# twice154/ofa-for-super-resolution

Measured on AMD Instinct MI355X. Metric: sr_training_images_per_sec_4x_64to256, higher is better.
Workload: dtype bf16; 1 GPU; OFA-SR S4 supernet 4x progressive shrinking (elastic kernel {3,5,7}, e=6, d=4, pd=2), LR 64x64 -> HR 256x256, fwd+bwd+Adam, train-mode BN; kernel_transform_mode=1, compat_reference_indexing=True, parallelism=dp1, per_gpu_batch=16, global_batch=16, grad_allreduce_bytes=0, launch=eager

## Files before the change

### ofa-for-super-resolution_amd/csrc/pwconv.hip

```cpp
#include <stdlib.h>
#include "ofasr_common.h"

namespace ofasr {

typedef __attribute__((ext_vector_type(16))) float f32x16;
typedef __attribute__((ext_vector_type(8))) __bf16 bf16x8;
typedef __attribute__((ext_vector_type(8))) _Float16 f16x8;
typedef __attribute__((ext_vector_type(4))) short s16x4;
typedef __attribute__((ext_vector_type(8))) short s16x8;
typedef __attribute__((address_space(3))) s16x4 lds_s16x4;

constexpr int PW_THREADS = 256;
constexpr int PW_TILE = 128;
constexpr int XROW16 = 320;
constexpr int XROW32 = 512;
constexpr int WROW16 = 128;
constexpr int WROW32 = 256;

template <typename T> struct Mma16;
template <> struct Mma16<bf16_t> {
    static __device__ __forceinline__ f32x16 run(s16x8 a, s16x8 b, f32x16 c) {
        return __builtin_amdgcn_mfma_f32_32x32x16_bf16(__builtin_bit_cast(bf16x8, a), __builtin_bit_cast(bf16x8, b),
                                                       c, 0, 0, 0);
    }
// ... 1177 lines not shown

template <typename T> struct Rows64 {
    static constexpr int NIT = Elem<T>::is16 ? 2 : 4;
    static constexpr int CPR = Elem<T>::is16 ? 8 : 16;
    static constexpr int EPC = Elem<T>::is16 ? 8 : 4;
    uint4 v[NIT];
    uint32_t ok;
};
template <typename T>
__device__ __forceinline__ void rows64_request(Rows64<T>& g, const T* __restrict__ base, int rows_total, int r0, int HW, int p0) {
    const int tid = threadIdx.x;
    g.ok = 0;
#pragma unroll
    for (int it = 0; it < Rows64<T>::NIT; ++it) {
        const int q = tid + it * PW_THREADS;
        const int r = q / Rows64<T>::CPR, ch = q % Rows64<T>::CPR;
        const int px = p0 + Rows64<T>::EPC * ch;
        const bool ok = r0 + r < rows_total && px < HW;
        g.v[it] = *reinterpret_cast<const uint4*>(base + (ok ? (long long)(r0 + r) * HW + px : 0));
        g.ok |= (ok ? 1u : 0u) << it;
    }
}
template <typename T>
__device__ __forceinline__ void rows64_deposit(char* Lt, const Rows64<T>& g) {
    const int tid = threadIdx.x;
#pragma unroll
    for (int it = 0; it < Rows64<T>::NIT; ++it) {
        const int q = tid + it * PW_THREADS;
        const int r = q / Rows64<T>::CPR, ch = q % Rows64<T>::CPR;
        const uint32_t m = (g.ok >> it) & 1u ? 0xffffffffu : 0u;
        *reinterpret_cast<uint4*>(Lt + wtile_chunk_off<T>(r, ch)) = make_uint4(g.v[it].x & m, g.v[it].y & m, g.v[it].z & m, g.v[it].w & m);
    }
}

template <typename T, bool ALIGNED>
__global__ void __launch_bounds__(PW_THREADS) pw_wgrad_kernel(const T* __restrict__ R, const T* __restrict__ S,
                                                              float* __restrict__ part, int MR, int NS, int HW,
                                                              int stages_per_img, int total_stages,
                                                              int stages_per_split) {
    constexpr int SUB = WgStage<T>::SUB;
    constexpr int TB = 64 * Elem<T>::wrow;
    __shared__ __attribute__((aligned(16))) char Rt[SUB * TB];
    __shared__ __attribute__((aligned(16))) char St[SUB * TB];
    const int r0 = blockIdx.x * 64, s0 = blockIdx.y * 64, z = blockIdx.z;
    const int lane = lane_id();
    const int wave = __builtin_amdgcn_readfirstlane((int)(threadIdx.x >> 6));
    const int c = lane & 31, h = lane >> 5;
    const int rb = wave & 1, sb = wave >> 1;
    f32x16 acc = zero16();
    const int q_lo = z * stages_per_split;
    const int q_hi = min(total_stages, q_lo + stages_per_split);
    auto multiply = [&]() {
#pragma unroll
        for (int sub = 0; sub < SUB; ++sub) {
            const char* Rs = Rt + sub * TB;
            const char* Ss = St + sub * TB;
            if constexpr (Elem<T>::is16) {
#pragma unroll
                for (int s = 0; s < 4; ++s) {
                    const s16x8 af = *reinterpret_cast<const s16x8*>(Rs + wtile_chunk_off<T>(32 * rb + c, 2 * s + h));
                    const s16x8 bf = *reinterpret_cast<const s16x8*>(Ss + wtile_chunk_off<T>(32 * sb + c, 2 * s + h));
                    acc = Mma16<T>::run(af, bf, acc);
                }
            } else {
#pragma unroll
                for (int s4 = 0; s4 < 8; ++s4) {
                    const float4 a4 = *reinterpret_cast<const float4*>(Rs + wtile_chunk_off<T>(32 * rb + c, 8 * h + s4));
                    const float4 b4 = *reinterpret_cast<const float4*>(Ss + wtile_chunk_off<T>(32 * sb + c, 8 * h + s4));
                    acc = __builtin_amdgcn_mfma_f32_32x32x2f32(a4.x, b4.x, acc, 0, 0, 0);
                    acc = __builtin_amdgcn_mfma_f32_32x32x2f32(a4.y, b4.y, acc, 0, 0, 0);
                    acc = __builtin_amdgcn_mfma_f32_32x32x2f32(a4.z, b4.z, acc, 0, 0, 0);
                    acc = __builtin_amdgcn_mfma_f32_32x32x2f32(a4.w, b4.w, acc, 0, 0, 0);
                }
            }
        }
    };
    if constexpr (ALIGNED) {
        Rows64<T> rg[SUB], sg[SUB];
        auto request = [&](int q) {
            const int n = q / stages_per_img;
            const int p0 = (q - n * stages_per_img) * (64 * SUB);
#pragma unroll
            for (int sub = 0; sub < SUB; ++sub) {
                rows64_request<T>(rg[sub], R + (long long)n * MR * HW, MR, r0, HW, p0 + 64 * sub);
                rows64_request<T>(sg[sub], S + (long long)n * NS * HW, NS, s0, HW, p0 + 64 * sub);
            }
        };
        if (q_lo < q_hi) request(q_lo);
        for (int q = q_lo; q < q_hi; ++q) {
            if (q > q_lo) __syncthreads();
#pragma unroll
            for (int sub = 0; sub < SUB; ++sub) {
                rows64_deposit<T>(Rt + sub * TB, rg[sub]);
                rows64_deposit<T>(St + sub * TB, sg[sub]);
            }
            __syncthreads();
            if (q + 1 < q_hi) request(q + 1);
            multiply();
        }
    } else {
        for (int q = q_lo; q < q_hi; ++q) {
            const int n = q / stages_per_img;
            const int p0 = (q - n * stages_per_img) * (64 * SUB);
            if (q > q_lo) __syncthreads();
#pragma unroll
            for (int sub = 0; sub < SUB; ++sub) {
                stage_rows64<T, ALIGNED>(Rt + sub * TB, R + (long long)n * MR * HW, MR, r0, HW, p0 + 64 * sub);
                stage_rows64<T, ALIGNED>(St + sub * TB, S + (long long)n * NS * HW, NS, s0, HW, p0 + 64 * sub);
            }
            __syncthreads();
            multiply();
        }
    }
    float* pz = part + (long long)z * MR * NS;
    const int sc = s0 + 32 * sb + c;
#pragma unroll
    for (int reg = 0; reg < 16; ++reg) {
        const int rr = r0 + 32 * rb + acc_row(reg, h);
        if (rr < MR && sc < NS) pz[(long long)rr * NS + sc] = acc[reg];
    }
}

constexpr int WR_ZL = 16;
__global__ void __launch_bounds__(64 * WR_ZL) pw_wgrad_reduce_kernel(const float* __restrict__ part,
                                                                     float* __restrict__ dw, int MR, int NS, int nsplit,
                                                                     long long sr, long long ss) {
    __shared__ float red[WR_ZL][64];
    const long long tot = (long long)MR * NS;
    const long long idx = (long long)blockIdx.x * 64 + (threadIdx.x & 63);
    const int zl = threadIdx.x >> 6;
    float a = 0.f;
    if (idx < tot) {
        int z = zl;
        for (; z + 3 * WR_ZL < nsplit; z += 4 * WR_ZL) {
            const float v0 = part[(long long)z * tot + idx], v1 = part[(long long)(z + WR_ZL) * tot + idx];
            const float v2 = part[(long long)(z + 2 * WR_ZL) * tot + idx], v3 = part[(long long)(z + 3 * WR_ZL) * tot + idx];
            a += (v0 + v1) + (v2 + v3);
        }
        for (; z < nsplit; z += WR_ZL) a += part[(long long)z * tot + idx];
    }
    red[zl][threadIdx.x & 63] = a;
    __syncthreads();
    if (zl == 0 && idx < tot) {
        float t = 0.f;
#pragma unroll
        for (int i = 0; i < WR_ZL; ++i) t += red[i][threadIdx.x];
        const long long r = idx / NS, sx = idx - r * NS;
        dw[r * sr + sx * ss] = t;
    }
}

constexpr int WD_RB = 3;
constexpr int WD_ROWS = 4 * WD_RB * 32, WD_COLS = 64;

struct WdPlan {
    int quads_per_img, total_quads, nsplit, MR, NS;
};

template <typename T, int XF = 0>
__global__ void __launch_bounds__(512) pw_wgrad_direct_kernel(const T* __restrict__ R, const T* __restrict__ S,
                                                              float* __restrict__ part, int MR, int NS, int HW,
                                                              WdPlan wp, InputXf xf = InputXf{}, BwdXf bx = BwdXf{}) {
    const int lane = lane_id();
    const int wave = __builtin_amdgcn_readfirstlane((int)(threadIdx.x >> 6));
    const int wr = wave & 3, wc = wave >> 2;
    const int c = lane & 31, h = lane >> 5;
    const int split = blockIdx.x;
    const int row0 = blockIdx.y * WD_ROWS + wr * (WD_RB * 32);
    const int col = blockIdx.z * WD_COLS + wc * 32 + c;
    if (row0 >= MR) return;
    f32x16 acc[WD_RB];
#pragma unroll
    for (int rb = 0; rb < WD_RB; ++rb) acc[rb] = zero16();
    const int q0 = (int)((long long)split * wp.total_quads / wp.nsplit);
    const int q1 = (int)((long long)(split + 1) * wp.total_quads / wp.nsplit);
    const bool cs = col < NS;
    const int colc = cs ? col : NS - 1;
    bool rs[WD_RB];
    int rowc[WD_RB];
#pragma unroll
    for (int rb = 0; rb < WD_RB; ++rb) {
        rs[rb] = row0 + 32 * rb + c < MR;
        rowc[rb] = rs[rb] ? row0 + 32 * rb + c : MR - 1;
    }
    float xsc[WD_RB], xmu[WD_RB], xb[WD_RB];
    float csc = 1.f, cmu = 0.f, cbb = 0.f;
    if constexpr (XF == 1) {
#pragma unroll
        for (int rb = 0; rb < WD_RB; ++rb) {
            xsc[rb] = xf.scale[rowc[rb]];
            xmu[rb] = xf.mean[rowc[rb]];
            xb[rb] = fmaf(xmu[rb], xsc[rb], xf.shift[rowc[rb]]);
        }
    }
    if constexpr (XF == 2) {
        csc = xf.scale[colc];
        cmu = xf.mean[colc];
        cbb = fmaf(cmu, csc, xf.shift[colc]);
    }
    float bka[WD_RB], bkbi[WD_RB];
    if constexpr (XF == 3) {
#pragma unroll
        for (int rb = 0; rb < WD_RB; ++rb) {
            xsc[rb] = bx.scale[rowc[rb]];
            xmu[rb] = bx.mean[rowc[rb]];
            xb[rb] = fmaf(xmu[rb], xsc[rb], bx.shift[rowc[rb]]);
            bka[rb] = bx.ka[rowc[rb]];
            bkbi[rb] = bx.kbi[rowc[rb]];
        }
    }
    long long rowoff[WD_RB];
#pragma unroll
    for (int rb = 0; rb < WD_RB; ++rb) rowoff[rb] = (long long)rowc[rb] * HW;
    const long long coloff = (long long)colc * HW;
    for (int q = q0; q < q1; ++q) {
        const int n = q / wp.quads_per_img;
        const int px = (q - n * wp.quads_per_img) * 64 + 32 * h;
        uint4 a[WD_RB][4], b[4];
        bool okp[4];
        int pxc[4];
#pragma unroll
        for (int j = 0; j < 4; ++j) {
            okp[j] = px + 8 * j < HW;
            pxc[j] = okp[j] ? px + 8 * j : 0;
        }
        const T* sp = S + (long long)n * NS * HW + coloff;
#pragma unroll
        for (int j = 0; j < 4; ++j) b[j] = *reinterpret_cast<const uint4*>(sp + pxc[j]);
        const T* rn = R + (long long)n * MR * HW;
#pragma unroll
        for (int rb = 0; rb < WD_RB; ++rb) {
#pragma unroll
            for (int j = 0; j < 4; ++j) {
                a[rb][j] = *reinterpret_cast<const uint4*>(rn + rowoff[rb] + pxc[j]);
            }
        }
        uint4 ya[XF == 3 ? WD_RB : 1][4];
        if constexpr (XF == 3) {
            const T* yn = reinterpret_cast<const T*>(bx.y) + (long long)n * MR * HW;
#pragma unroll
            for (int rb = 0; rb < WD_RB; ++rb) {
#pragma unroll
                for (int j = 0; j < 4; ++j)
                    ya[rb][j] = *reinterpret_cast<const uint4*>(yn + rowoff[rb] + pxc[j]);
            }
        }
#pragma unroll
        for (int j = 0; j < 4; ++j) {
            if constexpr (XF == 2) b[j] = xf_apply8_core<T>(b[j], csc, cmu, cbb);
            if (!(cs && okp[j])) b[j] = make_uint4(0, 0, 0, 0);
        }
#pragma unroll
        for (int rb = 0; rb < WD_RB; ++rb)
#pragma unroll
            for (int j = 0; j < 4; ++j) {
                if constexpr (XF == 1) a[rb][j] = xf_apply8_core<T>(a[rb][j], xsc[rb], xmu[rb], xb[rb]);
                if constexpr (XF == 3) a[rb][j] = bx_apply8<T>(a[rb][j], ya[rb][j], xmu[rb], xsc[rb], xb[rb], bka[rb], bkbi[rb]);
                if (!(rs[rb] && okp[j])) a[rb][j] = make_uint4(0, 0, 0, 0);
            }
#pragma unroll
        for (int j = 0; j < 4; ++j)
#pragma unroll
            for (int rb = 0; rb < WD_RB; ++rb)
                acc[rb] = Mma16<T>::run(__builtin_bit_cast(s16x8, a[rb][j]), __builtin_bit_cast(s16x8, b[j]), acc[rb]);
    }
    float* dst = part + (long long)split * MR * NS;
    if (cs) {
        float* p = dst + (long long)(row0 + 4 * h) * NS + col;
#pragma unroll
        for (int rb = 0; rb < WD_RB; ++rb)
#pragma unroll
            for (int reg = 0; reg < 16; ++reg) {
                const int r = row0 + 32 * rb + acc_row(reg, h);
                if (r < MR) *p = acc[rb][reg];
                p += (reg & 3) == 3 ? 5 * (long long)NS : (long long)NS;
            }
    }
}

static WdPlan wd_plan(int64_t N, int64_t Cin, int64_t Cout, int64_t HW) {
    WdPlan p;
    p.MR = (int)(Cout >= Cin ? Cout : Cin);
    p.NS = (int)(Cout >= Cin ? Cin : Cout);
    p.quads_per_img = (int)cdiv(HW, 64);
    p.total_quads = (int)(N * p.quads_per_img);
    const int64_t tiles = cdiv(p.MR, WD_ROWS) * cdiv(p.NS, WD_COLS);
    static const int blocks = [] { const char* e = getenv("OFASR_PW_WGRAD_BLOCKS"); const int v = e ? atoi(e) : 0; return v > 0 ? v : 256; }();
    int64_t want = blocks / (tiles > 0 ? tiles : 1);
    if (want > p.total_quads / 4) want = p.total_quads / 4;
    if (want < 1) want = 1;
    p.nsplit = (int)want;
    return p;
}


struct WdPlan32 {
    int units_per_img, total_units, nsplit, MR, NS;
};

__global__ void __launch_bounds__(512) pw_wgrad_direct_f32_kernel(const float* __restrict__ R, const float* __restrict__ S,
                                                                  float* __restrict__ part, int MR, int NS, int HW,
                                                                  WdPlan32 wp) {
    const int lane = lane_id();
    const int wave = __builtin_amdgcn_readfirstlane((int)(threadIdx.x >> 6));
    const int wr = wave & 3, wc = wave >> 2;
    const int c = lane & 31, h = lane >> 5;
    const int split = blockIdx.x;
    const int row0 = blockIdx.y * WD_ROWS + wr * (WD_RB * 32);
    const int col = blockIdx.z * WD_COLS + wc * 32 + c;
    if (row0 >= MR) return;
    f32x16 acc[WD_RB];
#pragma unroll
    for (int rb = 0; rb < WD_RB; ++rb) acc[rb] = zero16();
    const int u0 = (int)((long long)split * wp.total_units / wp.nsplit);
    const int u1 = (int)((long long)(split + 1) * wp.total_units / wp.nsplit);
    const bool cs = col < NS;
    const int colc = cs ? col : NS - 1;
    bool rs[WD_RB];
    long long rowoff[WD_RB];
#pragma unroll
    for (int rb = 0; rb < WD_RB; ++rb) {
        rs[rb] = row0 + 32 * rb + c < MR;
        rowoff[rb] = (long long)(rs[rb] ? row0 + 32 * rb + c : MR - 1) * HW;
    }
    float4 a[2][WD_RB][4], b[2][4];
    auto request = [&](int set, int u) {
        const int uc = u < u1 ? u : u1 - 1;
        const int n = uc / wp.units_per_img;
        const int px = (uc - n * wp.units_per_img) * 32 + 16 * h;
        int pxc[4];
#pragma unroll
        for (int j = 0; j < 4; ++j) pxc[j] = px + 4 * j < HW ? px + 4 * j : 0;
        const float* sp = S + ((long long)n * NS + colc) * HW;
        const float* rp = R + (long long)n * MR * HW;
#pragma unroll
        for (int j = 0; j < 4; ++j) b[set][j] = *reinterpret_cast<const float4*>(sp + pxc[j]);
#pragma unroll
        for (int rb = 0; rb < WD_RB; ++rb)
#pragma unroll
            for (int j = 0; j < 4; ++j) a[set][rb][j] = *reinterpret_cast<const float4*>(rp + rowoff[rb] + pxc[j]);
    };
    auto multiply = [&](int set, int u) {
        const int n = u / wp.units_per_img;
        const int px = (u - n * wp.units_per_img) * 32 + 16 * h;
        const bool live = u < u1;
#pragma unroll
        for (int j = 0; j < 4; ++j) {
            const bool ok = live && cs && px + 4 * j < HW;
            const float4 bv = ok ? b[set][j] : make_float4(0.f, 0.f, 0.f, 0.f);
#pragma unroll
            for (int rb = 0; rb < WD_RB; ++rb) {
                const float4 av = rs[rb] ? a[set][rb][j] : make_float4(0.f, 0.f, 0.f, 0.f);
                acc[rb] = __builtin_amdgcn_mfma_f32_32x32x2f32(av.x, bv.x, acc[rb], 0, 0, 0);
                acc[rb] = __builtin_amdgcn_mfma_f32_32x32x2f32(av.y, bv.y, acc[rb], 0, 0, 0);
                acc[rb] = __builtin_amdgcn_mfma_f32_32x32x2f32(av.z, bv.z, acc[rb], 0, 0, 0);
                acc[rb] = __builtin_amdgcn_mfma_f32_32x32x2f32(av.w, bv.w, acc[rb], 0, 0, 0);
            }
        }
    };
    if (u0 < u1) {
        request(0, u0);
        for (int u = u0; u < u1; u += 2) {
            request(1, u + 1);
            multiply(0, u);
            request(0, u + 2);
            multiply(1, u + 1);
        }
    }
    float* dst = part + (long long)split * MR * NS;
    if (cs) {
        float* p = dst + (long long)(row0 + 4 * h) * NS + col;
#pragma unroll
        for (int rb = 0; rb < WD_RB; ++rb)
#pragma unroll
            for (int reg = 0; reg < 16; ++reg) {
                const int r = row0 + 32 * rb + acc_row(reg, h);
                if (r < MR) *p = acc[rb][reg];
                p += (reg & 3) == 3 ? 5 * (long long)NS : (long long)NS;
            }
    }
}

static WdPlan32 wd_plan32(int64_t N, int64_t Cin, int64_t Cout, int64_t HW) {
    WdPlan32 p;
    p.MR = (int)(Cout >= Cin ? Cout : Cin);
    p.NS = (int)(Cout >= Cin ? Cin : Cout);
    p.units_per_img = (int)cdiv(HW, 32);
    p.total_units = (int)(N * p.units_per_img);
    const int64_t tiles = cdiv(p.MR, WD_ROWS) * cdiv(p.NS, WD_COLS);
    int64_t want = 256 / (tiles > 0 ? tiles : 1);
    if (want > p.total_units / 8) want = p.total_units / 8;
    if (want < 1) want = 1;
    p.nsplit = (int)want;
    return p;
}

struct WgradPlan {
    int stages_per_img, total_stages, nsplit, stages_per_split, MR, NS;
};

static WgradPlan wgrad_plan(int64_t N, int64_t Cin, int64_t Cout, int64_t HW, int sub) {
    WgradPlan p;
    p.MR = (int)(Cout >= Cin ? Cout : Cin);
    p.NS = (int)(Cout >= Cin ? Cin : Cout);
    p.stages_per_img = (int)cdiv(HW, 64 * sub);
    p.total_stages = (int)(N * p.stages_per_img);
    const int64_t tiles = cdiv(p.MR, 64) * cdiv(p.NS, 64);
    int64_t want = 512 / (tiles > 0 ? tiles : 1);
    if (want < 1) want = 1;
    if (want > p.total_stages) want = p.total_stages;
    if (want < 1) want = 1;
    p.stages_per_split = (int)cdiv(p.total_stages, want);
    if (p.stages_per_split < 1) p.stages_per_split = 1;
    p.nsplit = (int)cdiv(p.total_stages, p.stages_per_split);
    if (p.nsplit < 1) p.nsplit = 1;
    return p;
}

static bool aligned_for(const void* a, const void* b, int64_t HW, bool is16) {
    const uintptr_t bits = reinterpret_cast<uintptr_t>(a) | reinterpret_cast<uintptr_t>(b);
    return (bits & 15) == 0 && (HW % (is16 ? 8 : 4)) == 0;
}

template <typename T, bool AL, bool WV, bool XF = false>
static void launch_gemm_v(const void* x, WView wv, void* y, int64_t HW, int tiles_per_img, int total_tiles,
                          hipStream_t st, InputXf xf = InputXf{}, const void* addend = nullptr,
                          StatOut so = StatOut{nullptr, 0}, BnFold fold = BnFold{}) {
    if (wv.K <= 64) {
        if constexpr (Elem<T>::is16 && AL && WV && !XF) {
            static const bool slabs = [] { const char* e = getenv("OFASR_PW_FANOUT_SLABS"); return !(e && e[0] == '0'); }();
            const int nslab = wv.M / FO_ROWS;
            if (slabs && addend == nullptr && wv.K == 64 && wv.M % FO_ROWS == 0 && (nslab == 2 || nslab == 3) &&
                HW % PW_TILE == 0) {
                dim3 g1((unsigned)total_tiles);
#define OFASR_FO_SLABS(NS, ST)                                                                                       \
    OFASR_LAUNCH((pw_fanout_slabs_kernel<T, NS, ST>), g1, dim3(PW_THREADS), 0, st, (const T*)x, wv, (T*)y, (int)HW, \
                       tiles_per_img, so, BwdStatOut{})
                if (nslab == 3) { if (so.partial) OFASR_FO_SLABS(3, 1); else OFASR_FO_SLABS(3, 0); }
                else { if (so.partial) OFASR_FO_SLABS(2, 1); else OFASR_FO_SLABS(2, 0); }
#undef OFASR_FO_SLABS
                return;
            }
        }
        dim3 grid((unsigned)total_tiles, (unsigned)cdiv(wv.M, FO_ROWS));
        OFASR_LAUNCH((pw_fanout_kernel<T, AL, WV, XF>), grid, dim3(PW_THREADS), 0, st, (const T*)x, wv, (T*)y,
                           (int)HW, tiles_per_img, xf, (const T*)addend, so);
    } else {
        dim3 grid((unsigned)total_tiles, (unsigned)cdiv(wv.M, 64));
        if constexpr (Elem<T>::is16 && AL && WV) {
            static const bool fast_ok = [] { const char* e = getenv("OFASR_PW_FANIN_FAST"); return !(e && e[0] == '0'); }();
            const bool span32 = (long long)wv.K * HW < (1LL << 31) &&
                                (long long)wv.M * wv.sm + (long long)wv.K * wv.sk < (1LL << 31);
            if (fast_ok && wv.K % 4 == 0 && wv.M % 4 == 0 && span32)
                OFASR_LAUNCH((pw_fanin_pipe_kernel<T, XF, true>), grid, dim3(PW_THREADS), 0, st, (const T*)x, wv,
                                   (T*)y, (int)HW, tiles_per_img, (int)cdiv(wv.K, 64), xf, (const T*)addend, so, fold);
            else
                OFASR_LAUNCH((pw_fanin_pipe_kernel<T, XF, false>), grid, dim3(PW_THREADS), 0, st, (const T*)x, wv,
                                   (T*)y, (int)HW, tiles_per_img, (int)cdiv(wv.K, 64), xf, (const T*)addend, so, fold);
            return;
        }
        OFASR_LAUNCH((pw_fanin_kernel<T, AL, WV, XF>), grid, dim3(PW_THREADS), 0, st, (const T*)x, wv, (T*)y,
                           (int)HW, tiles_per_img, (int)cdiv(wv.K, 64), xf, (const T*)addend, so);
    }
}

template <typename T, bool XF = false>
static int launch_gemm(const char* name, const void* x, WView wv, void* y, int64_t N, int64_t HW, hipStream_t st,
                       InputXf xf = InputXf{}, const void* addend = nullptr, StatOut so = StatOut{nullptr, 0},
                       BnFold fold = BnFold{}) {
    constexpr bool is16 = Elem<T>::is16;
    const bool al = aligned_for(x, y, HW, is16);
    const long long ld = wv.sk == 1 ? wv.sm : wv.sk;
    const bool wvec = (reinterpret_cast<uintptr_t>(wv.w) & 15) == 0 && (ld % 4) == 0 && wv.K % 4 == 0 && wv.M % 4 == 0;
    const int tiles_per_img = (int)cdiv(HW, PW_TILE);
    const int64_t total64 = N * tiles_per_img;
    OFASR_REQUIRE(total64 <= INT32_MAX, OFASR_ERR_UNSUPPORTED, "%s: too many pixel tiles", name);
    const int total_tiles = (int)total64;
    {
        const double px = (double)N * (double)HW, es = (double)sizeof(T);
        prof_note(es * px * (wv.K + wv.M + (addend ? wv.M : 0)) + 4.0 * wv.K * wv.M, 2.0 * px * wv.K * wv.M);
    }
    if (so.partial)
        OFASR_REQUIRE(so.P == (wv.K <= 64 ? total_tiles : 2 * total_tiles), OFASR_ERR_INVALID_ARG,
                      "%s: statistics unit count %d does not match the launch", name, so.P);
    if constexpr (XF) {
        OFASR_REQUIRE(al && is16, OFASR_ERR_UNSUPPORTED, "%s: fused input transform needs aligned 16-bit tensors", name);
        if (fold.cp)
            OFASR_REQUIRE(wvec && wv.K > 64 && wv.K <= FOLD_KMAX, OFASR_ERR_UNSUPPORTED,
                          "%s: folded statistics need the pipelined fan-in kernel (64 < K <= %d)", name, FOLD_KMAX);
        if (wvec) launch_gemm_v<T, true, true, true>(x, wv, y, HW, tiles_per_img, total_tiles, st, xf, nullptr, so, fold);
        else launch_gemm_v<T, true, false, true>(x, wv, y, HW, tiles_per_img, total_tiles, st, xf, nullptr, so);
        return check_launch(name);
    }
    const bool al2 = al && (addend == nullptr || (reinterpret_cast<uintptr_t>(addend) & 15) == 0);
    if (al2 && wvec) launch_gemm_v<T, true, true>(x, wv, y, HW, tiles_per_img, total_tiles, st, InputXf{}, addend, so);
    else if (al2) launch_gemm_v<T, true, false>(x, wv, y, HW, tiles_per_img, total_tiles, st, InputXf{}, addend, so);
    else if (wvec) launch_gemm_v<T, false, true>(x, wv, y, HW, tiles_per_img, total_tiles, st, InputXf{}, addend, so);
    else launch_gemm_v<T, false, false>(x, wv, y, HW, tiles_per_img, total_tiles, st, InputXf{}, addend, so);
    return check_launch(name);
}

static int gemm_entry(const char* name, const void* x, WView wv, void* y, int64_t N, int64_t HW, int dtype,
                      void* stream, const void* addend = nullptr, StatOut so = StatOut{nullptr, 0}) {
    hipStream_t st = as_stream(stream);
    switch (dtype) {
        case OFASR_F32: return launch_gemm<float>(name, x, wv, y, N, HW, st, InputXf{}, addend, so);
        case OFASR_F16: return launch_gemm<f16_t>(name, x, wv, y, N, HW, st, InputXf{}, addend, so);
        default: return launch_gemm<bf16_t>(name, x, wv, y, N, HW, st, InputXf{}, addend, so);
    }
}

static int check_pw_args(const char* name, const void* a, const void* b, const void* c, int64_t ldw, int64_t N,
                         int64_t Cin, int64_t Cout, int64_t HW, int dtype) {
    OFASR_REQUIRE(a && b && c, OFASR_ERR_INVALID_ARG, "%s: null pointer", name);
    OFASR_REQUIRE(N >= 0 && Cin > 0 && Cout > 0 && HW >= 0, OFASR_ERR_INVALID_ARG,
                  "%s: bad shape N=%lld Cin=%lld Cout=%lld HW=%lld", name, (long long)N, (long long)Cin,
                  (long long)Cout, (long long)HW);
    OFASR_REQUIRE(ldw >= Cin, OFASR_ERR_INVALID_ARG, "%s: ldw=%lld < Cin=%lld", name, (long long)ldw, (long long)Cin);
    OFASR_REQUIRE(dtype == OFASR_F32 || dtype == OFASR_F16 || dtype == OFASR_BF16, OFASR_ERR_INVALID_ARG,
                  "%s: bad dtype %d", name, dtype);
    OFASR_REQUIRE(Cin <= 65536 && Cout <= 65536 && HW <= (1 << 30) && N <= (1 << 24), OFASR_ERR_UNSUPPORTED,
                  "%s: dimension too large", name);
    return OFASR_OK;
}

template <typename T, bool XF = false, bool BXM = false>
static int launch_wgrad(const char* name, const void* dy, const void* x, float* dw, int64_t ldw, int64_t N, int64_t Cin,
                        int64_t Cout, int64_t HW, float* ws, hipStream_t st, InputXf xf = InputXf{}, BwdXf bx = BwdXf{}) {
    const WgradPlan p = wgrad_plan(N, Cin, Cout, HW, WgStage<T>::SUB);
    const bool big_is_dy = Cout >= Cin;
    const T* R = (const T*)(big_is_dy ? dy : x);
    const T* S = (const T*)(big_is_dy ? x : dy);
    const long long sr = big_is_dy ? ldw : 1, ss = big_is_dy ? 1 : ldw;
    const bool al = aligned_for(dy, x, HW, Elem<T>::is16);
    prof_note((double)sizeof(T) * (double)N * (double)HW * (double)(Cin + Cout) + 4.0 * (double)Cin * (double)Cout,
              2.0 * (double)N * (double)HW * (double)Cin * (double)Cout);
    if constexpr (Elem<T>::is16) {
        if (al) {
            const WdPlan wp = wd_plan(N, Cin, Cout, HW);
            dim3 grid((unsigned)wp.nsplit, (unsigned)cdiv(wp.MR, WD_ROWS), (unsigned)cdiv(wp.NS, WD_COLS));
            if constexpr (XF) {
                if (big_is_dy)
                    OFASR_LAUNCH((pw_wgrad_direct_kernel<T, 2>), grid, dim3(512), 0, st, R, S, ws, wp.MR, wp.NS,
                                       (int)HW, wp, xf);
                else
                    OFASR_LAUNCH((pw_wgrad_direct_kernel<T, 1>), grid, dim3(512), 0, st, R, S, ws, wp.MR, wp.NS,
                                       (int)HW, wp, xf);
            } else if constexpr (BXM) {
                if (!big_is_dy) {
                    set_error("%s: the fused BN backward is implemented for the wide gradient operand (Cout >= Cin)", name);
                    return OFASR_ERR_UNSUPPORTED;
                }
                OFASR_LAUNCH((pw_wgrad_direct_kernel<T, 3>), grid, dim3(512), 0, st, R, S, ws, wp.MR, wp.NS, (int)HW, wp,
                             InputXf{}, bx);
            } else {
                OFASR_LAUNCH((pw_wgrad_direct_kernel<T>), grid, dim3(512), 0, st, R, S, ws, wp.MR, wp.NS, (int)HW,
                                   wp);
            }
            int rc = check_launch(name);
            if (rc) return rc;
            const long long tot = (long long)wp.MR * wp.NS;
            OFASR_LAUNCH(pw_wgrad_reduce_kernel, dim3((unsigned)cdiv(tot, 64)), dim3(64 * WR_ZL), 0, st, ws, dw, wp.MR,
                               wp.NS, wp.nsplit, sr, ss);
            return check_launch(name);
        }
    }
    if constexpr (XF || BXM) {
        set_error("%s: fused input transform needs the aligned 16-bit kernel", name);
        return OFASR_ERR_UNSUPPORTED;
    }
    if constexpr (!Elem<T>::is16) {
        static const bool f32_direct = [] { const char* e = getenv("OFASR_PW_WGRAD_F32_DIRECT"); return e && e[0] == '1'; }();
        if (al && f32_direct) {
            const WdPlan32 wp = wd_plan32(N, Cin, Cout, HW);
            dim3 grid((unsigned)wp.nsplit, (unsigned)cdiv(wp.MR, WD_ROWS), (unsigned)cdiv(wp.NS, WD_COLS));
            OFASR_LAUNCH(pw_wgrad_direct_f32_kernel, grid, dim3(512), 0, st, (const float*)R, (const float*)S, ws, wp.MR, wp.NS,
                         (int)HW, wp);
            int rc = check_launch(name);
            if (rc) return rc;
            const long long tot = (long long)wp.MR * wp.NS;
            OFASR_LAUNCH(pw_wgrad_reduce_kernel, dim3((unsigned)cdiv(tot, 64)), dim3(64 * WR_ZL), 0, st, ws, dw, wp.MR, wp.NS,
                         wp.nsplit, sr, ss);
            return check_launch(name);
        }
    }
    dim3 grid((unsigned)cdiv(p.MR, 64), (unsigned)cdiv(p.NS, 64), (unsigned)p.nsplit);
    if (al)
        OFASR_LAUNCH((pw_wgrad_kernel<T, true>), grid, dim3(PW_THREADS), 0, st, R, S, ws, p.MR, p.NS, (int)HW,
                           p.stages_per_img, p.total_stages, p.stages_per_split);
    else
        OFASR_LAUNCH((pw_wgrad_kernel<T, false>), grid, dim3(PW_THREADS), 0, st, R, S, ws, p.MR, p.NS, (int)HW,
                           p.stages_per_img, p.total_stages, p.stages_per_split);
    int rc = check_launch(name);
    if (rc) return rc;
    const long long tot = (long long)p.MR * p.NS;
    OFASR_LAUNCH(pw_wgrad_reduce_kernel, dim3((unsigned)cdiv(tot, 64)), dim3(64 * WR_ZL), 0, st, ws, dw, p.MR, p.NS,
                       p.nsplit, sr, ss);
    return check_launch(name);
}

int pwconv_dgrad_add(const void* dy, const float* w, int64_t ldw, void* dx, const void* addend, int64_t N, int64_t Cin,
                     int64_t Cout, int64_t HW, int dtype, void* stream) {
    const char* name = "pwconv_dgrad_add";
    int rc = check_pw_args(name, dy, w, dx, ldw, N, Cin, Cout, HW, dtype);
    if (rc) return rc;
    OFASR_REQUIRE(addend != nullptr, OFASR_ERR_INVALID_ARG, "%s: null addend", name);
    if (N * HW == 0) return OFASR_OK;
    WView wv{w, 1, ldw, (int)Cin, (int)Cout};
    return gemm_entry(name, dy, wv, dx, N, HW, dtype, stream, addend);
}

bool pwconv_dgrad_bx_supported(const void* da, const void* y, const void* dx, const void* addend, const float* w,
                               int64_t ldw, int64_t Cin, int64_t Cout, int64_t HW, int dtype) {
    if (dtype != OFASR_F16 && dtype != OFASR_BF16) return false;
    const uintptr_t bits = reinterpret_cast<uintptr_t>(da) | reinterpret_cast<uintptr_t>(y) | reinterpret_cast<uintptr_t>(dx) |
                           reinterpret_cast<uintptr_t>(addend) | reinterpret_cast<uintptr_t>(w);
    static const bool fast_ok = [] { const char* e = getenv("OFASR_PW_FANIN_FAST"); return !(e && e[0] == '0'); }();
    return fast_ok && (bits & 15) == 0 && HW % 8 == 0 && ldw % 4 == 0 && Cin % 4 == 0 && Cout % 4 == 0 && Cout > 64 &&
           Cout <= FOLD_KMAX && Cout * HW < (1LL << 31) && (Cin + Cout) * ldw < (1LL << 31);
}

template <typename T>
static int launch_dgrad_bx(const char* name, const void* da, WView wv, void* dx, const void* addend, int64_t N, int64_t HW,
                           BwdXf bx, hipStream_t st) {
    const int tiles_per_img = (int)cdiv(HW, PW_TILE);
    const int64_t total64 = N * tiles_per_img;
    OFASR_REQUIRE(total64 <= INT32_MAX, OFASR_ERR_UNSUPPORTED, "%s: too many pixel tiles", name);
    {
        const double px = (double)N * (double)HW, es = (double)sizeof(T);
        prof_note(es * px * (2.0 * wv.K + wv.M + (addend ? wv.M : 0)) + 4.0 * wv.K * wv.M, 2.0 * px * wv.K * wv.M);
    }
    dim3 grid((unsigned)total64, (unsigned)cdiv(wv.M, 64));
    OFASR_LAUNCH((pw_fanin_pipe_kernel<T, false, true, true>), grid, dim3(PW_THREADS), 0, st, (const T*)da, wv, (T*)dx,
                 (int)HW, tiles_per_img, (int)cdiv(wv.K, 64), InputXf{}, (const T*)addend, StatOut{nullptr, 0}, BnFold{}, bx);
    return check_launch(name);
}

int pwconv_dgrad_add_bx(const void* da, const float* w, int64_t ldw, void* dx, const void* addend, int64_t N, int64_t Cin,
                        int64_t Cout, int64_t HW, int dtype, BwdXf bx, void* stream) {
    const char* name = "pwconv_dgrad_add_bx";
    int rc = check_pw_args(name, da, w, dx, ldw, N, Cin, Cout, HW, dtype);
    if (rc) return rc;
    OFASR_REQUIRE(bx.y && bx.mean && bx.scale && bx.shift &&
                      ((bx.ka && bx.kbi) || (bx.fold_partial && bx.fold_invstd && bx.fold_P > 0 && bx.fold_C == Cout)),
                  OFASR_ERR_INVALID_ARG, "%s: null transform", name);
    OFASR_REQUIRE(pwconv_dgrad_bx_supported(da, bx.y, dx, addend, w, ldw, Cin, Cout, HW, dtype), OFASR_ERR_UNSUPPORTED,
                  "%s: needs the pipelined fan-in kernel (aligned 16-bit tensors, 64 < Cout <= %d)", name, FOLD_KMAX);
    if (N * HW == 0) return OFASR_OK;
    WView wv{w, 1, ldw, (int)Cin, (int)Cout};
    hipStream_t st = as_stream(stream);
    if (dtype == OFASR_F16) return launch_dgrad_bx<f16_t>(name, da, wv, dx, addend, N, HW, bx, st);
    return launch_dgrad_bx<bf16_t>(name, da, wv, dx, addend, N, HW, bx, st);
}

bool pwconv_xf_supported(const void* x, const void* y, int64_t HW, int dtype) {
    return (dtype == OFASR_F16 || dtype == OFASR_BF16) && aligned_for(x, y, HW, true);
}

bool pwconv_dgrad_bstat_supported(const void* dy, const void* y, const void* dx, const float* w, int64_t ldw, int64_t Cin,
                                  int64_t Cout, int64_t HW, int dtype) {
    const bool wvec = (reinterpret_cast<uintptr_t>(w) & 15) == 0 && (ldw % 4) == 0;
    return (dtype == OFASR_F16 || dtype == OFASR_BF16) && aligned_for(dy, dx, HW, true) &&
           (reinterpret_cast<uintptr_t>(y) & 15) == 0 && wvec && Cout == 64 && (Cin == 2 * FO_ROWS || Cin == 3 * FO_ROWS) &&
           HW % PW_TILE == 0;
}

template <typename T>
static int launch_dgrad_bstat(const void* dy, WView wv, void* dx, int64_t N, int64_t HW, BwdStatOut bs, hipStream_t st) {
    const int tiles_per_img = (int)(HW / PW_TILE);
    const int total_tiles = (int)(N * tiles_per_img);
    const double px = (double)N * (double)HW;
    prof_note(2.0 * px * (wv.K + 2.0 * wv.M) + 4.0 * wv.K * wv.M, 2.0 * px * wv.K * wv.M);
    if (wv.M == 3 * FO_ROWS)
        OFASR_LAUNCH((pw_fanout_slabs_kernel<T, 3, 2>), dim3((unsigned)total_tiles), dim3(PW_THREADS), 0, st, (const T*)dy, wv,
                     (T*)dx, (int)HW, tiles_per_img, StatOut{nullptr, 0}, bs);
    else
        OFASR_LAUNCH((pw_fanout_slabs_kernel<T, 2, 2>), dim3((unsigned)total_tiles), dim3(PW_THREADS), 0, st, (const T*)dy, wv,
                     (T*)dx, (int)HW, tiles_per_img, StatOut{nullptr, 0}, bs);
    return check_launch("pwconv_dgrad_bstat");
}

int pwconv_dgrad_bstat(const void* dy, const float* w, int64_t ldw, void* dx, int64_t N, int64_t Cin, int64_t Cout,
                       int64_t HW, int dtype, BwdStatOut bs, void* stream) {
    const char* name = "pwconv_dgrad_bstat";
    int rc = check_pw_args(name, dy, w, dx, ldw, N, Cin, Cout, HW, dtype);
    if (rc) return rc;
    OFASR_REQUIRE(bs.y && bs.mean && bs.scale && bs.shift && bs.partial, OFASR_ERR_INVALID_ARG, "%s: null pointer", name);
    OFASR_REQUIRE(pwconv_dgrad_bstat_supported(dy, bs.y, dx, w, ldw, Cin, Cout, HW, dtype), OFASR_ERR_UNSUPPORTED,
                  "%s: shape outside the slab-walk kernel", name);
    OFASR_REQUIRE(N * (HW / PW_TILE) <= INT32_MAX && bs.P == (int)(N * (HW / PW_TILE)), OFASR_ERR_INVALID_ARG,
                  "%s: unit count %d does not match the launch", name, bs.P);
    WView wv{w, 1, ldw, (int)Cin, (int)Cout};
    hipStream_t st = as_stream(stream);
// ... 154 lines not shown
```

Before: 2712 images/s.

## Restructure pointwise wgrad kernel: per-block K-split across waves with LDS reduction

Each block now covers a 96x64 output tile, and its 8 waves split the pixel (K) range among themselves. Each wave computes a 3x2 grid of MFMA tiles, so every loaded A/B fragment feeds more MFMAs. Partial sums are reduced across waves in LDS before wave 0 writes them out. The grid becomes 1D, with block indices arranged so the 8 splits of a tile land on different XCDs. For the BN-backward variant, the S loads are deferred behind a sched_barrier to lower register pressure. The cost is a larger accumulator footprint and extra LDS reduction barriers, which may lower occupancy.

```diff
diff --git a/ofa-for-super-resolution_amd/csrc/pwconv.hip b/ofa-for-super-resolution_amd/csrc/pwconv.hip
--- a/ofa-for-super-resolution_amd/csrc/pwconv.hip
+++ b/ofa-for-super-resolution_amd/csrc/pwconv.hip
@@ -1353,56 +1353,71 @@
 
 constexpr int WD_RB = 3;
 constexpr int WD_ROWS = 4 * WD_RB * 32, WD_COLS = 64;
+constexpr int WS_RB = 3, WS_CB = 2;
+constexpr int WS_ROWS = 32 * WS_RB, WS_COLS = 32 * WS_CB;
+constexpr int WS_WAVES = 8;
 
 struct WdPlan {
-    int quads_per_img, total_quads, nsplit, MR, NS;
+    int quads_per_img, total_quads, nsplit, MR, NS, row_tiles, col_tiles;
 };
 
 template <typename T, int XF = 0>
 __global__ void __launch_bounds__(512) pw_wgrad_direct_kernel(const T* __restrict__ R, const T* __restrict__ S,
                                                               float* __restrict__ part, int MR, int NS, int HW,
                                                               WdPlan wp, InputXf xf = InputXf{}, BwdXf bx = BwdXf{}) {
+    __shared__ float4 red[4 * WS_RB * 4 * 64];
     const int lane = lane_id();
     const int wave = __builtin_amdgcn_readfirstlane((int)(threadIdx.x >> 6));
-    const int wr = wave & 3, wc = wave >> 2;
     const int c = lane & 31, h = lane >> 5;
-    const int split = blockIdx.x;
-    const int row0 = blockIdx.y * WD_ROWS + wr * (WD_RB * 32);
-    const int col = blockIdx.z * WD_COLS + wc * 32 + c;
-    if (row0 >= MR) return;
-    f32x16 acc[WD_RB];
-#pragma unroll
-    for (int rb = 0; rb < WD_RB; ++rb) acc[rb] = zero16();
+    const int G = wp.row_tiles * wp.col_tiles;
+    const int xcd = blockIdx.x & 7, jb = blockIdx.x >> 3;
+    const int group = jb % G, split = (jb / G) * 8 + xcd;
+    if (split >= wp.nsplit) return;
+    const int row0 = (group % wp.row_tiles) * WS_ROWS;
+    const int col0 = (group / wp.row_tiles) * WS_COLS;
+    f32x16 acc[WS_RB][WS_CB];
+#pragma unroll
+    for (int rb = 0; rb < WS_RB; ++rb)
+#pragma unroll
+        for (int cb = 0; cb < WS_CB; ++cb) acc[rb][cb] = zero16();
     const int q0 = (int)((long long)split * wp.total_quads / wp.nsplit);
     const int q1 = (int)((long long)(split + 1) * wp.total_quads / wp.nsplit);
-    const bool cs = col < NS;
-    const int colc = cs ? col : NS - 1;
-    bool rs[WD_RB];
-    int rowc[WD_RB];
-#pragma unroll
-    for (int rb = 0; rb < WD_RB; ++rb) {
+    bool cs[WS_CB];
+    int colc[WS_CB];
+#pragma unroll
+    for (int cb = 0; cb < WS_CB; ++cb) {
+        cs[cb] = col0 + 32 * cb + c < NS;
+        colc[cb] = cs[cb] ? col0 + 32 * cb + c : NS - 1;
+    }
+    bool rs[WS_RB];
+    int rowc[WS_RB];
+#pragma unroll
+    for (int rb = 0; rb < WS_RB; ++rb) {
         rs[rb] = row0 + 32 * rb + c < MR;
         rowc[rb] = rs[rb] ? row0 + 32 * rb + c : MR - 1;
     }
-    float xsc[WD_RB], xmu[WD_RB], xb[WD_RB];
-    float csc = 1.f, cmu = 0.f, cbb = 0.f;
+    float xsc[WS_RB], xmu[WS_RB], xb[WS_RB];
+    float csc[WS_CB], cmu[WS_CB], cbb[WS_CB];
     if constexpr (XF == 1) {
 #pragma unroll
-        for (int rb = 0; rb < WD_RB; ++rb) {
+        for (int rb = 0; rb < WS_RB; ++rb) {
             xsc[rb] = xf.scale[rowc[rb]];
             xmu[rb] = xf.mean[rowc[rb]];
             xb[rb] = fmaf(xmu[rb], xsc[rb], xf.shift[rowc[rb]]);
         }
     }
     if constexpr (XF == 2) {
-        csc = xf.scale[colc];
-        cmu = xf.mean[colc];
-        cbb = fmaf(cmu, csc, xf.shift[colc]);
-    }
-    float bka[WD_RB], bkbi[WD_RB];
+#pragma unroll
+        for (int cb = 0; cb < WS_CB; ++cb) {
+            csc[cb] = xf.scale[colc[cb]];
+            cmu[cb] = xf.mean[colc[cb]];
+            cbb[cb] = fmaf(cmu[cb], csc[cb], xf.shift[colc[cb]]);
+        }
+    }
+    float bka[WS_RB], bkbi[WS_RB];
     if constexpr (XF == 3) {
 #pragma unroll
-        for (int rb = 0; rb < WD_RB; ++rb) {
+        for (int rb = 0; rb < WS_RB; ++rb) {
             xsc[rb] = bx.scale[rowc[rb]];
             xmu[rb] = bx.mean[rowc[rb]];
             xb[rb] = fmaf(xmu[rb], xsc[rb], bx.shift[rowc[rb]]);
@@ -1410,14 +1425,15 @@
             bkbi[rb] = bx.kbi[rowc[rb]];
         }
     }
-    long long rowoff[WD_RB];
-#pragma unroll
-    for (int rb = 0; rb < WD_RB; ++rb) rowoff[rb] = (long long)rowc[rb] * HW;
-    const long long coloff = (long long)colc * HW;
-    for (int q = q0; q < q1; ++q) {
+    long long rowoff[WS_RB], coloff[WS_CB];
+#pragma unroll
+    for (int rb = 0; rb < WS_RB; ++rb) rowoff[rb] = (long long)rowc[rb] * HW;
+#pragma unroll
+    for (int cb = 0; cb < WS_CB; ++cb) coloff[cb] = (long long)colc[cb] * HW;
+    for (int q = q0 + wave; q < q1; q += WS_WAVES) {
         const int n = q / wp.quads_per_img;
         const int px = (q - n * wp.quads_per_img) * 64 + 32 * h;
-        uint4 a[WD_RB][4], b[4];
+        uint4 a[WS_RB][4], b[WS_CB][4];
         bool okp[4];
         int pxc[4];
 #pragma unroll
@@ -1425,57 +1441,101 @@
             okp[j] = px + 8 * j < HW;
             pxc[j] = okp[j] ? px + 8 * j : 0;
         }
-        const T* sp = S + (long long)n * NS * HW + coloff;
-#pragma unroll
-        for (int j = 0; j < 4; ++j) b[j] = *reinterpret_cast<const uint4*>(sp + pxc[j]);
+        const T* sn = S + (long long)n * NS * HW;
+        auto request_s = [&]() {
+#pragma unroll
+            for (int cb = 0; cb < WS_CB; ++cb)
+#pragma unroll
+                for (int j = 0; j < 4; ++j) b[cb][j] = *reinterpret_cast<const uint4*>(sn + coloff[cb] + pxc[j]);
+        };
+        if constexpr (XF != 3) request_s();
         const T* rn = R + (long long)n * MR * HW;
 #pragma unroll
-        for (int rb = 0; rb < WD_RB; ++rb) {
+        for (int rb = 0; rb < WS_RB; ++rb) {
 #pragma unroll
             for (int j = 0; j < 4; ++j) {
                 a[rb][j] = *reinterpret_cast<const uint4*>(rn + rowoff[rb] + pxc[j]);
             }
         }
-        uint4 ya[XF == 3 ? WD_RB : 1][4];
+        uint4 ya[XF == 3 ? WS_RB : 1][4];
         if constexpr (XF == 3) {
             const T* yn = reinterpret_cast<const T*>(bx.y) + (long long)n * MR * HW;
 #pragma unroll
-            for (int rb = 0; rb < WD_RB; ++rb) {
+            for (int rb = 0; rb < WS_RB; ++rb) {
 #pragma unroll
                 for (int j = 0; j < 4; ++j)
                     ya[rb][j] = *reinterpret_cast<const uint4*>(yn + rowoff[rb] + pxc[j]);
             }
         }
 #pragma unroll
-        for (int j = 0; j < 4; ++j) {
-            if constexpr (XF == 2) b[j] = xf_apply8_core<T>(b[j], csc, cmu, cbb);
-            if (!(cs && okp[j])) b[j] = make_uint4(0, 0, 0, 0);
-        }
-#pragma unroll
-        for (int rb = 0; rb < WD_RB; ++rb)
+        for (int rb = 0; rb < WS_RB; ++rb)
 #pragma unroll
             for (int j = 0; j < 4; ++j) {
                 if constexpr (XF == 1) a[rb][j] = xf_apply8_core<T>(a[rb][j], xsc[rb], xmu[rb], xb[rb]);
                 if constexpr (XF == 3) a[rb][j] = bx_apply8<T>(a[rb][j], ya[rb][j], xmu[rb], xsc[rb], xb[rb], bka[rb], bkbi[rb]);
                 if (!(rs[rb] && okp[j])) a[rb][j] = make_uint4(0, 0, 0, 0);
             }
+        if constexpr (XF == 3) {
+            __builtin_amdgcn_sched_barrier(0);
+            request_s();
+        }
+#pragma unroll
+        for (int cb = 0; cb < WS_CB; ++cb)
+#pragma unroll
+            for (int j = 0; j < 4; ++j) {
+                if constexpr (XF == 2) b[cb][j] = xf_apply8_core<T>(b[cb][j], csc[cb], cmu[cb], cbb[cb]);
+                if (!(cs[cb] && okp[j])) b[cb][j] = make_uint4(0, 0, 0, 0);
+            }
 #pragma unroll
         for (int j = 0; j < 4; ++j)
 #pragma unroll
-            for (int rb = 0; rb < WD_RB; ++rb)
-                acc[rb] = Mma16<T>::run(__builtin_bit_cast(s16x8, a[rb][j]), __builtin_bit_cast(s16x8, b[j]), acc[rb]);
+            for (int cb = 0; cb < WS_CB; ++cb)
+#pragma unroll
+                for (int rb = 0; rb < WS_RB; ++rb)
+                    acc[rb][cb] = Mma16<T>::run(__builtin_bit_cast(s16x8, a[rb][j]), __builtin_bit_cast(s16x8, b[cb][j]),
+                                                acc[rb][cb]);
     }
     float* dst = part + (long long)split * MR * NS;
-    if (cs) {
-        float* p = dst + (long long)(row0 + 4 * h) * NS + col;
-#pragma unroll
-        for (int rb = 0; rb < WD_RB; ++rb)
-#pragma unroll
-            for (int reg = 0; reg < 16; ++reg) {
-                const int r = row0 + 32 * rb + acc_row(reg, h);
-                if (r < MR) *p = acc[rb][reg];
-                p += (reg & 3) == 3 ? 5 * (long long)NS : (long long)NS;
-            }
+#pragma unroll
+    for (int cb = 0; cb < WS_CB; ++cb) {
+#pragma unroll
+        for (int st = 4; st >= 1; st >>= 1) {
+            if (wave >= st && wave < 2 * st) {
+                float4* slot = red + (wave & 3) * (WS_RB * 4 * 64) + lane;
+#pragma unroll
+                for (int rb = 0; rb < WS_RB; ++rb)
+#pragma unroll
+                    for (int g = 0; g < 4; ++g)
+                        slot[(rb * 4 + g) * 64] = make_float4(acc[rb][cb][4 * g], acc[rb][cb][4 * g + 1],
+                                                              acc[rb][cb][4 * g + 2], acc[rb][cb][4 * g + 3]);
+            }
+            lds_barrier();
+            if (wave < st) {
+                const float4* slot = red + ((wave + st) & 3) * (WS_RB * 4 * 64) + lane;
+#pragma unroll
+                for (int rb = 0; rb < WS_RB; ++rb)
+#pragma unroll
+                    for (int g = 0; g < 4; ++g) {
+                        const float4 v = slot[(rb * 4 + g) * 64];
+                        acc[rb][cb][4 * g] += v.x;
+                        acc[rb][cb][4 * g + 1] += v.y;
+                        acc[rb][cb][4 * g + 2] += v.z;
+                        acc[rb][cb][4 * g + 3] += v.w;
+                    }
+            }
+        }
+        if (cb + 1 < WS_CB) lds_barrier();
+        if (wave == 0 && cs[cb]) {
+            float* p = dst + (long long)(row0 + 4 * h) * NS + col0 + 32 * cb + c;
+#pragma unroll
+            for (int rb = 0; rb < WS_RB; ++rb)
+#pragma unroll
+                for (int reg = 0; reg < 16; ++reg) {
+                    const int r = row0 + 32 * rb + acc_row(reg, h);
+                    if (r < MR) *p = acc[rb][cb][reg];
+                    p += (reg & 3) == 3 ? 5 * (long long)NS : (long long)NS;
+                }
+        }
     }
 }
 
@@ -1485,10 +1545,12 @@
     p.NS = (int)(Cout >= Cin ? Cin : Cout);
     p.quads_per_img = (int)cdiv(HW, 64);
     p.total_quads = (int)(N * p.quads_per_img);
-    const int64_t tiles = cdiv(p.MR, WD_ROWS) * cdiv(p.NS, WD_COLS);
+    p.row_tiles = (int)cdiv(p.MR, WS_ROWS);
+    p.col_tiles = (int)cdiv(p.NS, WS_COLS);
+    const int64_t tiles = (int64_t)p.row_tiles * p.col_tiles;
     static const int blocks = [] { const char* e = getenv("OFASR_PW_WGRAD_BLOCKS"); const int v = e ? atoi(e) : 0; return v > 0 ? v : 256; }();
     int64_t want = blocks / (tiles > 0 ? tiles : 1);
-    if (want > p.total_quads / 4) want = p.total_quads / 4;
+    if (want > p.total_quads / WS_WAVES) want = p.total_quads / WS_WAVES;
     if (want < 1) want = 1;
     p.nsplit = (int)want;
     return p;
@@ -1739,7 +1801,7 @@
     if constexpr (Elem<T>::is16) {
         if (al) {
             const WdPlan wp = wd_plan(N, Cin, Cout, HW);
-            dim3 grid((unsigned)wp.nsplit, (unsigned)cdiv(wp.MR, WD_ROWS), (unsigned)cdiv(wp.NS, WD_COLS));
+            dim3 grid((unsigned)(8 * wp.row_tiles * wp.col_tiles * cdiv(wp.nsplit, 8)));
             if constexpr (XF) {
                 if (big_is_dy)
                     OFASR_LAUNCH((pw_wgrad_direct_kernel<T, 2>), grid, dim3(512), 0, st, R, S, ws, wp.MR, wp.NS,
```

Result: no change. 2693 images/s (-0.7%).
